# graphdeco-inria/nerfshop

Hardware: AMD Instinct MI355X
Metric: render_msamples_per_s_1080p (higher is better)
Workload: dtype f16 storage / f32 accumulate (MFMA), f32 marching+compositing; 1 GPU; lego-like snapshot 1920x1080, one cage edit (BASELINE configs[2]/[4]); samples_per_frame=25213758, frames_in_flight=1, cell_records=levels 0..11, 9.2 GB (nrs_model_set_cell_cache default)

## Files before the change

nerfshop_amd/csrc/nrs_api_edit.cpp:

```cpp
#include "nrs_host.h"

#include <cmath>
#include <cstdio>
#include <cstring>
#include <limits>
#include <memory>
#include <new>

using namespace nrs;

static void box_of(const float* v, uint32_t n, Box3& b) {
	const float inf = std::numeric_limits<float>::infinity();
	for (int k = 0; k < 3; ++k) { b.mn[k] = inf; b.mx[k] = -inf; }
	for (uint32_t i = 0; i < n; ++i)
		for (int k = 0; k < 3; ++k) {
			b.mn[k] = std::fmin(b.mn[k], v[3 * i + k]);
			b.mx[k] = std::fmax(b.mx[k], v[3 * i + k]);
		}
}
static void warp_box(const Box3& b, const Box3& aabb, Box3& out) {
	for (int k = 0; k < 3; ++k) {
		const float diag = aabb.mx[k] - aabb.mn[k];
		out.mn[k] = (b.mn[k] - aabb.mn[k]) / diag;
		out.mx[k] = (b.mx[k] - aabb.mn[k]) / diag;
// ... 78 lines not shown
			for (int a = 0; a < 3; ++a) { f[a] = w[a] << shift; f[4 + a] = (w[3 + a] - w[a] + 1) << shift; }
			f[7] = shift;
			budget -= cells;
			base += (uint32_t)cells;
			any = true;
			break;
		}
	}
	if (!any) { memset(de.fine_win, 0, sizeof(de.fine_win)); return NRS_OK; }
	const uint32_t n_cells = base, n_padded = (n_cells + 4095u) / 4096u * 4096u;
	if (n_padded > e->fine_cells_cap || (want_head && !e->d_fine_head.get())) {
		e->d_fine_off.reset(); e->d_fine_counts.reset(); e->d_fine_head.reset();
		e->fine_cells_cap = 0;
		const size_t cap = std::min<size_t>(kFineMaxCells, (size_t)n_padded + n_padded / 4 + 4095) / 4096 * 4096;
		HIP_TRY(e->d_fine_off.alloc(cap + 1));
		HIP_TRY(e->d_fine_counts.alloc(cap));
		if (want_head) HIP_TRY(e->d_fine_head.alloc(cap));
		e->fine_cells_cap = cap;
	}
	NRS_LAUNCH(launch_fine_count_scan(de, n_cells, e->d_fine_counts.get(), e->d_fine_tiles.get(), e->d_fine_off.get(), (uint32_t*)e->d_fine_win.get() + kCascades * 8, s));
	uint32_t n_idx = 0;
	HIP_TRY(hipMemcpyAsync(&n_idx, e->d_fine_win.get() + kCascades * 8, 4, hipMemcpyDeviceToHost, s));
	HIP_TRY(hipStreamSynchronize(s));
	if ((size_t)n_idx > e->fine_idx_cap || !e->d_fine_idx.get()) {
		e->d_fine_idx.reset();
		e->fine_idx_cap = 0;
		const size_t cap = std::max<size_t>((size_t)n_idx + n_idx / 2, 1024);
		HIP_TRY(e->d_fine_idx.alloc(cap));
		e->fine_idx_cap = cap;
	}
	NRS_LAUNCH(launch_fine_fill(de, n_cells, e->d_fine_off.get(), e->d_fine_idx.get(), want_head ? e->d_fine_head.get() : nullptr, s));
	e->fine_n_idx = n_idx;
	de.fine_off = e->d_fine_off.get();
	de.fine_idx = e->d_fine_idx.get();
	de.fine_head = want_head ? e->d_fine_head.get() : nullptr;
	static const bool log_fine = dev_knob("NRS_FINE_LOG") != nullptr;
	if (log_fine) fprintf(stderr, "[nrs fine lut] %u fine cells, %u entries (the LUT holds %u), subdivision per cascade %d %d %d %d %d, head words %s\n", n_cells, n_idx, e->lut_n_idx, de.fine_win[0][7],
	                      de.fine_win[1][7], de.fine_win[2][7], de.fine_win[3][7], de.fine_win[4][7], de.fine_head ? "yes" : "no");
	return NRS_OK;
}
static int rebuild_after_vertices(nrs_edit* e, hipStream_t s, bool build_fine_now = false) {
	NRS_TRY(ensure_build_scratch(e));
	NRS_LAUNCH(launch_bbox(e->n_vertices, e->d_verts.get(), (float*)e->d_scratch.get(), s));
	NRS_TRY(build_lut_on_device(e, e->d_verts.get(), nullptr, s));
	if (e->d_rot.get()) NRS_LAUNCH(launch_local_rotations(e->n_tets, e->d_verts.get(), e->de.orig, e->de.tets, e->d_rot.get(), e->d_mapback.get(), s));
	NRS_LAUNCH(launch_tet_planes(e->n_tets, e->d_verts.get(), e->de.tets, e->d_planes.get(), s));
	if (build_fine_now) NRS_TRY(build_fine_lut(e, s));
	else {
		e->de.fine_off = nullptr;
		e->de.fine_idx = nullptr;
		e->de.fine_head = nullptr;
		memset(e->de.fine_win, 0, sizeof(e->de.fine_win));
		e->fine_stale = true;
		e->renders_since_move = 0;
	}
	uint32_t host[8];
	HIP_TRY(hipMemcpyAsync(host, e->d_scratch.get(), sizeof(host), hipMemcpyDeviceToHost, s));
	HIP_TRY(hipStreamSynchronize(s));
	memcpy(e->de.bbox.mn, host, 12);
	memcpy(e->de.bbox.mx, host + 3, 12);
	warp_box(e->de.bbox, e->de.aabb, e->de.warped_bbox);
// ... 283 lines not shown
```

nerfshop_amd/csrc/nrs_api_render.cpp:

```cpp
#include "nrs_host.h"

#include <array>
#include <cmath>
#include <cstdio>
#include <cstdlib>
#include <cstring>

using namespace nrs;

extern "C" {

static int tile_geometry(const nrs_render_params& p, uint32_t team, uint32_t& tiles_x, uint32_t& owned, uint32_t& n_packets, uint32_t& ppt_x) {
	const uint32_t W = (uint32_t)p.resolution[0], H = (uint32_t)p.resolution[1];
	const uint32_t pw = team >= 16 ? 2u : (team >= 4 ? 4u : 8u), ph = 64u / team / pw;
	if (p.tile_size == 0) {
		tiles_x = (W + pw - 1) / pw;
		owned = 1;
		ppt_x = 0;
		n_packets = tiles_x * ((H + ph - 1) / ph);
		return NRS_OK;
	}
	if (p.tile_size % 8) return fail(NRS_ERR_INVALID_ARG, "tile_size must be a multiple of 8");
	tiles_x = tile_pitch(W, p.tile_size);
	const uint32_t tiles_y = (H + p.tile_size - 1) / p.tile_size, total = tiles_x * tiles_y;
// ... 173 lines not shown
		}
		ctx->counters_clean[slot] = true;
	}
	HIP_TRY(hipEventRecord(ctx->slot_done[slot], s));
	ctx->slot_stream[slot] = s;
	ctx->slot_used[slot] = true;
	return NRS_OK;
}

static int report_wave_log(nrs_ctx* ctx, const RenderCounters& c) {
	static const char* names[8] = {"fill", "refill", "setup+warp", "gather", "sh+mlp", "composite+march+shade", "-", "exit"};
	unsigned long long tot = 0;
	for (int i = 0; i < 8; ++i) if (i != 6) tot += c.phase_cycles[i];
	fprintf(stderr, "[nrs phases] samples=%llu", (unsigned long long)c.n_samples);
	for (int i = 0; i < 8; ++i)
		if (c.phase_cycles[i] && i != 6) fprintf(stderr, " %s=%.1f%%", names[i], 100.0 * (double)c.phase_cycles[i] / (double)tot);
	fprintf(stderr, " | mean wave lifetime = %.1f%% of the longest (%.2f Mcycles)", 100.0 * ((double)tot / 4096.0) / (double)c.phase_cycles[6], (double)c.phase_cycles[6] / 1e6);
	fprintf(stderr, "\n");
	fprintf(stderr, "[nrs walk] fill: %llu lane iterations in %llu wave trips (%.1f lanes busy per trip); march: %llu lane iterations in %llu wave trips "
	        "(%.1f lanes/trip), %llu of %llu rounds needed > 1 trip; live lanes per round %.1f\n",
	        c.walk[0], c.walk[1], c.walk[1] ? (double)c.walk[0] / (double)c.walk[1] : 0.0, c.walk[2], c.walk[3],
	        c.walk[3] ? (double)c.walk[2] / (double)c.walk[3] : 0.0, c.walk[6], c.walk[4], c.walk[4] ? (double)c.walk[5] / (double)c.walk[4] : 0.0);
	if (c.walk[8])
		fprintf(stderr, "[nrs cage scan] %llu samples inside a deformed box (%.1f %% of the samples), %llu of them found a tet; rounds with such a sample: %llu of %llu (%.1f %%); "
		        "candidates tested %llu (%.2f per sample in the box), scan wave trips %llu (%.2f per round that scans)\n",
		        c.walk[8], 100.0 * (double)c.walk[8] / (double)std::max<unsigned long long>(c.n_samples, 1), c.walk[12], c.walk[9], c.walk[4], 100.0 * (double)c.walk[9] / (double)std::max<unsigned long long>(c.walk[4], 1),
		        c.walk[10], (double)c.walk[10] / (double)c.walk[8], c.walk[11], (double)c.walk[11] / (double)std::max<unsigned long long>(c.walk[9], 1));
	std::vector<unsigned long long> wl(8192 * 4);
	HIP_TRY(hipMemcpy(wl.data(), ctx->d_wave_log.get(), wl.size() * 8, hipMemcpyDeviceToHost));
	if (const char* dump = dev_knob("NRS_WAVE_LOG_FILE")) {
		if (FILE* f = fopen(dump, "wb")) { fwrite(wl.data(), 8, wl.size(), f); fclose(f); }
	}
	std::vector<std::array<unsigned long long, 4>> rec;
	unsigned long long t0min = ~0ull;
	for (size_t i = 0; i < 8192; ++i) if (wl[4 * i]) t0min = std::min(t0min, wl[4 * i + 3] >> 32);
	for (size_t i = 0; i < 8192; ++i)
		if (wl[4 * i]) {
			const unsigned long long wall = wl[4 * i + 3] & 0xffffffffull, start = (wl[4 * i + 3] >> 32) - t0min;
			const unsigned long long rq = (wl[4 * i + 1] >> 16) & 0xffff, tq = (wl[4 * i + 1] >> 32) + start;
			rec.push_back({wall + start, (wl[4 * i + 1] & 0xffffull) | (rq << 16) | (tq << 32), wl[4 * i + 2] & 0xffffull, wl[4 * i + 2] >> 56});
		}
	std::sort(rec.begin(), rec.end());
	if (!rec.empty()) {
		auto pr = [&](const char* tag, size_t i) {
			fprintf(stderr, "   %s: end=%.1f us, queue found empty at %.1f us, rounds=%llu (%llu after that), packets=%llu, xcc=%llu\n", tag, rec[i][0] / 100.0,
			        (rec[i][1] >> 32) / 100.0, rec[i][1] & 0xffff, (rec[i][1] & 0xffff) - ((rec[i][1] >> 16) & 0xffff), rec[i][2], rec[i][3]);
		};
		double mean = 0;
		for (auto& r : rec) mean += (double)r[0];
// ... 154 lines not shown
```

nerfshop_amd/csrc/nrs_cage.hip:

```cpp
#include <hip/hip_runtime.h>
#include "nrs_internal.h"
#include "nrs_launch.h"
#include "nrs_device.cuh"
#include "nrs_scan.cuh"
#include "nrs_svd3.h"

namespace nrs {


constexpr uint32_t kCells = kGridVol * kCascades;
constexpr uint32_t kScanTile = 4096;
static_assert(kCells % kScanTile == 0, "scan tiles must cover the cell array exactly");
constexpr uint32_t kScanTiles = kCells / kScanTile;
static_assert(kFineMaxCells % kScanTile == 0 && kFineScanTiles == kFineMaxCells / kScanTile, "fine look-up table: scan tiles");

__global__ void mvc_apply_kernel(uint32_t n_points, uint32_t n_cv, const float* __restrict__ weights, const float* __restrict__ cage,
                                 float* __restrict__ points) {
	const uint32_t i = blockIdx.x * blockDim.x + threadIdx.x;
	if (i >= n_points) return;
	f3 p = mk3(0.f, 0.f, 0.f);
	const float* w = weights + (size_t)i * n_cv;
	for (uint32_t v = 0; v < n_cv; ++v) {
		const float wv = w[v];
		p = p + mk3(wv * cage[3 * v], wv * cage[3 * v + 1], wv * cage[3 * v + 2]);
	}
	points[3 * i] = p.x; points[3 * i + 1] = p.y; points[3 * i + 2] = p.z;
}

// ... 393 lines not shown
	float R[9];
	svd3::tet_rotation(o, d, R);
	for (int k = 0; k < 9; ++k) out[9 * (size_t)i + k] = R[k];
	if (mapback)
		for (int k = 0; k < 9; ++k) mapback[24 * (size_t)i + 12 + k] = R[k];
}
__global__ void tet_mapback_kernel(uint32_t n_tets, const float* __restrict__ org, const uint32_t* __restrict__ tets, const float* __restrict__ rot, float* __restrict__ mapback) {
	const uint32_t i = blockIdx.x * blockDim.x + threadIdx.x;
	if (i >= n_tets) return;
	const uint4 tv = reinterpret_cast<const uint4*>(tets)[i];
	const f3 v[4] = {ld3(org, tv.x), ld3(org, tv.y), ld3(org, tv.z), ld3(org, tv.w)};
	float out[24];
	for (int f = 0; f < 4; ++f) { out[3 * f] = v[f].x; out[3 * f + 1] = v[f].y; out[3 * f + 2] = v[f].z; }
	for (int k = 0; k < 9; ++k) out[12 + k] = rot ? rot[9 * (size_t)i + k] : 0.f;
	for (int k = 21; k < 24; ++k) out[k] = 0.f;
	float4* dst = reinterpret_cast<float4*>(mapback) + 6 * (size_t)i;
	for (int q = 0; q < 6; ++q) dst[q] = make_float4(out[4 * q], out[4 * q + 1], out[4 * q + 2], out[4 * q + 3]);
}

__global__ void tet_planes_kernel(uint32_t n_tets, const float* __restrict__ verts, const uint32_t* __restrict__ tets, float* __restrict__ planes) {
	const uint32_t i = blockIdx.x * blockDim.x + threadIdx.x;
	if (i >= n_tets) return;
	const uint4 tv = reinterpret_cast<const uint4*>(tets)[i];
	const f3 v[4] = {ld3(verts, tv.x), ld3(verts, tv.y), ld3(verts, tv.z), ld3(verts, tv.w)};
	float out[32];
	uint32_t signs = 0;
	for (int f = 0; f < 4; ++f) {
		const f3 v1 = v[f], v2 = v[(f + 1) & 3], v3 = v[(f + 2) & 3], v4 = v[(f + 3) & 3];
		const f3 normal = cross3(v2 - v1, v3 - v1);
		const float dotV4 = dot3(normal, v4 - v1);
		out[3 * f] = v1.x; out[3 * f + 1] = v1.y; out[3 * f + 2] = v1.z;
		out[12 + 3 * f] = normal.x; out[12 + 3 * f + 1] = normal.y; out[12 + 3 * f + 2] = normal.z;
		signs |= (__float_as_uint(dotV4) >> 31) << f;
	}
	out[24] = __uint_as_float(signs);
	for (int k = 25; k < 32; ++k) out[k] = 0.f;
	float4* dst = reinterpret_cast<float4*>(planes) + 8 * (size_t)i;
	for (int q = 0; q < 8; ++q) dst[q] = make_float4(out[4 * q], out[4 * q + 1], out[4 * q + 2], out[4 * q + 3]);
}

__global__ __launch_bounds__(256) void fine_window_kernel(const uint32_t* __restrict__ offsets, int32_t* __restrict__ win) {
	__shared__ int32_t red[8];
	if (threadIdx.x < 8) red[threadIdx.x] = threadIdx.x < 3 ? 0x7fffffff : (threadIdx.x < 6 ? -1 : 0);
	__syncthreads();
	const uint32_t first = (blockIdx.x * blockDim.x + threadIdx.x) * 16u;
	uint32_t o[17];
	#pragma unroll
	for (int q = 0; q < 4; ++q) { const uint4 v = reinterpret_cast<const uint4*>(offsets + first)[q]; o[4 * q] = v.x; o[4 * q + 1] = v.y; o[4 * q + 2] = v.z; o[4 * q + 3] = v.w; }
	o[16] = offsets[first + 16];
	if (o[0] != o[16]) {
		int32_t lo[3] = {0x7fffffff, 0x7fffffff, 0x7fffffff}, hi[3] = {-1, -1, -1}, cells = 0, longest = 0;
		#pragma unroll
		for (uint32_t k = 0; k < 16; ++k) {
			if (o[k + 1] != o[k]) {
				const uint32_t m = (first + k) % kGridVol;
				const int32_t c[3] = {(int32_t)morton3D_invert(m), (int32_t)morton3D_invert(m >> 1), (int32_t)morton3D_invert(m >> 2)};
				for (int a = 0; a < 3; ++a) { lo[a] = min(lo[a], c[a]); hi[a] = max(hi[a], c[a]); }
				++cells;
				longest = max(longest, (int32_t)(o[k + 1] - o[k]));
			}
		}
		for (int a = 0; a < 3; ++a) { atomicMin(&red[a], lo[a]); atomicMax(&red[3 + a], hi[a]); }
		atomicAdd(&red[6], cells);
		atomicMax(&red[7], longest);
	}
	__syncthreads();
	if (threadIdx.x < 8 && red[6] != 0) {
		int32_t* dst = win + (blockIdx.x * blockDim.x * 16u / kGridVol) * 8 + threadIdx.x;
		if (threadIdx.x < 3) atomicMin(dst, red[threadIdx.x]);
		else if (threadIdx.x < 6 || threadIdx.x == 7) atomicMax(dst, red[threadIdx.x]);
		else atomicAdd(dst, red[6]);
	}
}
__device__ __forceinline__ bool tet_may_contain_box(const float* __restrict__ r, const float c[3], const float h[3]) {
	const uint32_t signs = __float_as_uint(r[24]);
	bool may = true;
	#pragma unroll
	for (int f = 0; f < 4; ++f) {
		float dc = 0.f, rad = 0.f, err = 0.f;
		#pragma unroll
		for (int i = 0; i < 3; ++i) {
			const float n = r[12 + 3 * f + i], d = c[i] - r[3 * f + i];
			dc = fmaf(n, d, dc);
			rad = fmaf(fabsf(n), h[i], rad);
			err = fmaf(fabsf(n), fabsf(d) + h[i], err);
		}
		const float slack = fmaf(err, 20.0f / 16777216.0f, 1e-30f);
		may = may && (((signs >> f) & 1u) ? !(dc - rad > slack) : !(dc + rad < -slack));
	}
	return may;
}
template <bool FILL>
__global__ __launch_bounds__(256) void fine_lists_kernel(const DeviceEdit e, uint32_t* __restrict__ counts, const uint32_t* __restrict__ fine_off,
                                                         uint32_t* __restrict__ fine_idx, uint2* __restrict__ fine_head) {
	uint32_t w = blockIdx.x * (blockDim.x >> 6) + (threadIdx.x >> 6);
	const uint32_t lane = threadIdx.x & 63u;
	uint32_t level = kCascades;
	#pragma unroll
	for (uint32_t c = 0; c < kCascades; ++c) {
		const int32_t* f = e.fine_win[c];
		const uint32_t n_par = (f[4] == 0 || (uint32_t)f[7] > 2u) ? 0u : ((uint32_t)f[4] >> f[7]) * ((uint32_t)f[5] >> f[7]) * ((uint32_t)f[6] >> f[7]);
		if (level == kCascades) { if (w < n_par) level = c; else w -= n_par; }
	}
	if (level == kCascades) return;
	const uint32_t S = (uint32_t)e.fine_win[level][7], sub = 1u << S;
	const uint32_t ex = (uint32_t)e.fine_win[level][4], ey = (uint32_t)e.fine_win[level][5];
	const uint32_t px = ex >> S, py = ey >> S;
	const uint32_t cx = w % px, cy = (w / px) % py, cz = w / (px * py);
	const uint32_t lx = ((uint32_t)e.fine_win[level][0] >> S) + cx, ly = ((uint32_t)e.fine_win[level][1] >> S) + cy, lz = ((uint32_t)e.fine_win[level][2] >> S) + cz;
	const uint32_t parent = level * kGridVol + morton3D(lx, ly, lz);
	const uint32_t j0 = e.lut_off[parent], j1 = e.lut_off[parent + 1];
	const bool owner = lane < sub * sub * sub;
	const uint32_t sx = lane & (sub - 1u), sy = (lane >> S) & (sub - 1u), sz = lane >> (2u * S);
	const uint32_t rx = (cx << S) + sx, ry = (cy << S) + sy, rz = (cz << S) + sz;
	const uint32_t cell = (uint32_t)e.fine_win[level][3] + (rz * ey + ry) * ex + rx;
	if (j0 == j1) {
		if (!FILL && owner) counts[cell] = 0u;
		if (FILL && owner && fine_head) fine_head[cell] = make_uint2(0u, 0u);
		return;
	}
	const uint32_t res = kGrid << S;
	const double scale = (double)(1u << level), margin = 2e-6 * scale;
	const uint32_t f[3] = {(uint32_t)e.fine_win[level][0] + rx, (uint32_t)e.fine_win[level][1] + ry, (uint32_t)e.fine_win[level][2] + rz};
	float c[3], h[3];
	bool border = false;
	#pragma unroll
	for (int i = 0; i < 3; ++i) {
		const double lo = 0.5 + ((double)f[i] / (double)res - 0.5) * scale - margin, hi = 0.5 + ((double)(f[i] + 1) / (double)res - 0.5) * scale + margin;
		c[i] = (float)(0.5 * (lo + hi));
		h[i] = (float)(0.5 * (hi - lo));
		border = border || f[i] == 0 || f[i] >= res - 1;
	}
	uint32_t n = 0, wpos = (FILL && owner) ? fine_off[cell] : 0u;
	const uint32_t wpos0 = wpos;
	uint32_t first = 0u;
	for (uint32_t b = j0; b < j1; b += 64u) {
		const uint32_t mine = b + lane < j1 ? e.lut_idx[b + lane] : 0u;
		const uint32_t nb = min(64u, j1 - b);
		float4 cur[7], nxt[7];
		{
			const float4* q = reinterpret_cast<const float4*>(e.planes) + 8 * (size_t)(uint32_t)__builtin_amdgcn_readlane((int)mine, 0);
			#pragma unroll
			for (int i = 0; i < 7; ++i) cur[i] = q[i];
		}
		for (uint32_t k = 0; k < nb; ++k) {
			const uint32_t t = (uint32_t)__builtin_amdgcn_readlane((int)mine, (int)k);
			const uint32_t t_next = (uint32_t)__builtin_amdgcn_readlane((int)mine, (int)min(k + 1u, nb - 1u));
			{
				const float4* q = reinterpret_cast<const float4*>(e.planes) + 8 * (size_t)t_next;
				#pragma unroll
				for (int i = 0; i < 7; ++i) nxt[i] = q[i];
			}
			const float* r = reinterpret_cast<const float*>(cur);
			if ((border || tet_may_contain_box(r, c, h)) && owner) {
				if (FILL) { fine_idx[wpos++] = t; if (n == 0) first = t; }
				++n;
			}
			#pragma unroll
			for (int i = 0; i < 7; ++i) cur[i] = nxt[i];
		}
	}
	if (!FILL && owner) counts[cell] = n;
	if (FILL && owner && fine_head) fine_head[cell] = make_uint2(wpos0, first | (n << kFineHeadTetBits));
}

int launch_mvc_apply(uint32_t n_points, uint32_t n_cv, const float* d_weights, const float* d_cage, float* d_points, void* stream) {
	hipLaunchKernelGGL(mvc_apply_kernel, dim3((n_points + 127) / 128), dim3(128), 0, (hipStream_t)stream, n_points, n_cv, d_weights, d_cage, d_points);
	NRS_LAUNCH_CHECK("mvc_apply_kernel launch");
	return NRS_OK;
}
int launch_poisson_interpolate(uint32_t n_points, uint32_t n_cv, const float* d_gamma, const float* d_per_cage, float* d_shs, float* d_out_density, float* d_res_density, void* stream) {
	hipLaunchKernelGGL(poisson_interpolate_kernel, dim3((n_points + 63) / 64), dim3(64), 0, (hipStream_t)stream, n_points, n_cv, d_gamma, d_per_cage, d_shs, d_out_density, d_res_density);
	NRS_LAUNCH_CHECK("poisson_interpolate_kernel launch");
	return NRS_OK;
}
int launch_bbox(uint32_t n, const float* d_verts, float* d_out6, void* stream) {
	hipLaunchKernelGGL(bbox_kernel, dim3(1), dim3(256), 0, (hipStream_t)stream, n, d_verts, d_out6);
	NRS_LAUNCH_CHECK("bbox_kernel launch");
	return NRS_OK;
}
int launch_lut_count_scan(uint32_t n_tets, const float* d_verts, const uint32_t* d_tets, uint32_t* d_counts, uint32_t* d_tile_sums,
                          uint32_t* d_offsets, uint32_t* d_total, unsigned long long* d_hit_masks, float cells0, void* stream) {
	hipStream_t s = (hipStream_t)stream;
	launch_tet_mark<false>(n_tets, cells0, d_verts, d_tets, d_counts, nullptr, nullptr, d_hit_masks, s);
	const int status = launch_cell_scan(kScanTiles, d_counts, d_tile_sums, d_offsets, d_total, s);
	if (status != NRS_OK) return status;
// ... 71 lines not shown
```

nerfshop_amd/csrc/nrs_device.cuh:

```cuda
#pragma once
#include <hip/hip_runtime.h>
#include "nrs_internal.h"

namespace nrs {

struct f3 { float x, y, z; };
__device__ __forceinline__ f3 mk3(float x, float y, float z) { return f3{x, y, z}; }
__device__ __forceinline__ f3 operator+(f3 a, f3 b) { return {a.x + b.x, a.y + b.y, a.z + b.z}; }
__device__ __forceinline__ f3 operator-(f3 a, f3 b) { return {a.x - b.x, a.y - b.y, a.z - b.z}; }
__device__ __forceinline__ f3 operator*(f3 a, float s) { return {a.x * s, a.y * s, a.z * s}; }
__device__ __forceinline__ f3 operator*(float s, f3 a) { return {s * a.x, s * a.y, s * a.z}; }
__device__ __forceinline__ float sum3(float a, float b, float c) { return a + (b + c); }
__device__ __forceinline__ float dot3(f3 a, f3 b) { return sum3(a.x * b.x, a.y * b.y, a.z * b.z); }
__device__ __forceinline__ f3 mat3_mul(const float* M, f3 v) {
	return {sum3(M[0] * v.x, M[3] * v.y, M[6] * v.z), sum3(M[1] * v.x, M[4] * v.y, M[7] * v.z), sum3(M[2] * v.x, M[5] * v.y, M[8] * v.z)};
}
__device__ __forceinline__ f3 cross3(f3 a, f3 b) { return {a.y * b.z - a.z * b.y, a.z * b.x - a.x * b.z, a.x * b.y - a.y * b.x}; }

__device__ __forceinline__ bool box_contains(const Box3& b, f3 p) {
	return p.x >= b.mn[0] && p.x <= b.mx[0] && p.y >= b.mn[1] && p.y <= b.mx[1] && p.z >= b.mn[2] && p.z <= b.mx[2];
}

#define NRS_SQRT3 1.73205080757f
#define NRS_MIN_STEP (NRS_SQRT3 / 1024)
#define NRS_MAX_STEP (NRS_MIN_STEP * (1 << (kCascades - 1)) * 1024 / kGrid)
// ... 574 lines not shown
	       same_side_tet(v4, v1, v2, v3, p);
}
__device__ __forceinline__ void bary_tet(f3 a, f3 b, f3 c, f3 d, f3 p, float out[4]) {
	f3 vap = p - a, vbp = p - b, vab = b - a, vac = c - a, vad = d - a, vbc = c - b, vbd = d - b;
	float va6 = scalar_tp(vbp, vbd, vbc);
	float vb6 = scalar_tp(vap, vac, vad);
	float vc6 = scalar_tp(vap, vad, vab);
	float vd6 = scalar_tp(vap, vab, vac);
	float v6 = (float)(1. / (double)scalar_tp(vab, vac, vad));
	out[0] = va6 * v6; out[1] = vb6 * v6; out[2] = vc6 * v6; out[3] = vd6 * v6;
}
template <typename T>
__device__ __forceinline__ const NRS_GLOBAL T* gp(const T* p) { return (const NRS_GLOBAL T*)p; }
__device__ __forceinline__ f3 ld3(const float* __restrict__ a, uint32_t i) {
	typedef float f3a __attribute__((ext_vector_type(3), aligned(4)));
	const f3a v = *(const NRS_GLOBAL f3a*)(gp(a) + 3 * (size_t)i);
	return {v.x, v.y, v.z};
}

__device__ __forceinline__ bool point_in_tet_rec(const float* __restrict__ recs, uint32_t t, f3 p) {
	typedef float f4n __attribute__((ext_vector_type(4)));
	const NRS_GLOBAL f4n* q = gp(reinterpret_cast<const f4n*>(recs)) + 8 * (size_t)t;
	const f4n v0 = q[0], v1 = q[1], v2 = q[2], n0 = q[3], n1 = q[4], n2 = q[5], sg = q[6];
	const float d0 = dot3(mk3(n0.x, n0.y, n0.z), p - mk3(v0.x, v0.y, v0.z));
	const float d1 = dot3(mk3(n0.w, n1.x, n1.y), p - mk3(v0.w, v1.x, v1.y));
	const float d2 = dot3(mk3(n1.z, n1.w, n2.x), p - mk3(v1.z, v1.w, v2.x));
	const float d3 = dot3(mk3(n2.y, n2.z, n2.w), p - mk3(v2.y, v2.z, v2.w));
	const uint32_t got = (__float_as_uint(d0) >> 31) | ((__float_as_uint(d1) >> 31) << 1) | ((__float_as_uint(d2) >> 31) << 2) | ((__float_as_uint(d3) >> 31) << 3);
	return got == __float_as_uint(sg.x);
}
__device__ __forceinline__ uint32_t scan_entries_for_tet(const DeviceEdit& e, const NRS_GLOBAL uint32_t* lut_idx, uint32_t j0, uint32_t j1, uint32_t t, f3 p, uint32_t* n_tested) {
	uint32_t found = 0xffffffffu;
	#pragma unroll 1
	for (uint32_t j = j0; j < j1; ++j) {
		const uint32_t t_next = lut_idx[min(j + 1, j1 - 1)];
		if (n_tested) ++*n_tested;
		if (point_in_tet_rec(e.planes, t, p)) { found = t; break; }
		t = t_next;
	}
	return found;
}
__device__ __forceinline__ uint32_t scan_list_for_tet(const DeviceEdit& e, const uint32_t* __restrict__ off, const uint32_t* __restrict__ idx, uint32_t cell, f3 p, uint32_t* n_tested = nullptr) {
	const NRS_GLOBAL uint32_t* lut_off = gp(off);
	const NRS_GLOBAL uint32_t* lut_idx = gp(idx);
	const uint32_t j0 = lut_off[cell], j1 = lut_off[cell + 1];
	if (j0 >= j1) return 0xffffffffu;
	return scan_entries_for_tet(e, lut_idx, j0, j1, lut_idx[j0], p, n_tested);
}
__device__ __forceinline__ uint32_t scan_cell_for_tet(const DeviceEdit& e, uint32_t cell, f3 p, uint32_t* n_tested = nullptr) { return scan_list_for_tet(e, e.lut_off, e.lut_idx, cell, p, n_tested); }
__device__ __forceinline__ uint32_t scan_fine_cell_for_tet(const DeviceEdit& e, uint32_t cell, f3 p, uint32_t* n_tested = nullptr) {
	typedef uint32_t u2n __attribute__((ext_vector_type(2)));
	const u2n head = *reinterpret_cast<const NRS_GLOBAL u2n*>(gp(e.fine_head) + cell);
	const uint32_t n = head.y >> kFineHeadTetBits;
	return scan_entries_for_tet(e, gp(e.fine_idx), head.x, head.x + n, head.y & ((1u << kFineHeadTetBits) - 1u), p, n_tested);
}
template <bool SHORT = true>
__device__ __forceinline__ uint32_t find_tet(const DeviceEdit& e, f3 u, const uint32_t* __restrict__ march_lds, uint32_t* n_tested = nullptr) {
	const int level = mip_from_pos(u);
	if (e.fine_off) {
		typedef int32_t i4n __attribute__((ext_vector_type(4)));
		i4n lo, ext;
		const int level_u = __builtin_amdgcn_readfirstlane(level);
		if (SHORT && __all(level == level_u)) {
			const NRS_CONSTANT i4n* win = (const NRS_CONSTANT i4n*)reinterpret_cast<const i4n*>(&e.fine_win[0][0]) + 2 * level_u;
			lo = win[0]; ext = win[1];
		} else {
			const NRS_GLOBAL i4n* win = gp(reinterpret_cast<const i4n*>(&e.fine_win[0][0])) + 2 * level;
			lo = win[0]; ext = win[1];
		}
		const float mip_scale = ldexpf(1.0f, -level);
		f3 q = u - mk3(0.5f, 0.5f, 0.5f);
		q = q * mip_scale;
		q = q + mk3(0.5f, 0.5f, 0.5f);
		if (ext.w != kFinePlain) {
			const int fres_i = (int)(kGrid << ext.w);
			const float fres = (float)fres_i;
			const int hi = fres_i - 1;
// ... 57 lines not shown
				f4n r0 = {0.f, 0.f, 0.f, 0.f}, r1 = {0.f, 0.f, 0.f, 0.f};
				float r2 = 0.f;
				if (rotate) { r0 = mq[3]; r1 = mq[4]; r2 = reinterpret_cast<const NRS_GLOBAL float*>(mq)[20]; }
				f3 canon = bc[0] * mk3(o0.x, o0.y, o0.z) + bc[1] * mk3(o0.w, o1.x, o1.y);
				canon = canon + bc[2] * mk3(o1.z, o1.w, o2.x);
				canon = canon + bc[3] * mk3(o2.y, o2.z, o2.w);
				wpos = e.diag_pow2 ? mk3((canon.x - e.aabb.mn[0]) * e.inv_diag[0], (canon.y - e.aabb.mn[1]) * e.inv_diag[1], (canon.z - e.aabb.mn[2]) * e.inv_diag[2])
				                   : warp_position(canon, e.aabb);
				if (rotate) {
					const f3 ud = unwarp_direction(wdir);
					const float R[9] = {r0.x, r0.y, r0.z, r0.w, r1.x, r1.y, r1.z, r1.w, r2};
					const f3 rd = mat3_mul(R, ud);
					wdir = warp_direction(rd);
				}
			}
			in_deformed = true;
		}
	}
	bool empty = false;
	if (!(with_dir && e.copy)) {
		if (!in_deformed && box_contains(e.orig_warped_bbox, wpos)) {
			const f3 u = unwarp_position(wpos, e.aabb);
			const int level = mip_from_pos(u);
			const uint32_t pos_idx = cascaded_grid_idx_at(u, (uint32_t)level);
			empty = gp(e.orig_bitfield)[pos_idx / 8 + (kGridVol * (uint32_t)level) / 8] & (1 << (pos_idx % 8));
		}
	}
	return empty;
}

__device__ __forceinline__ bool affine_contains(const AffineBox& b, f3 p) {
	const f3 q = p - mk3(b.mn[0], b.mn[1], b.mn[2]);
	const float du = dot3(mk3(b.u[0], b.u[1], b.u[2]), q), dv = dot3(mk3(b.v[0], b.v[1], b.v[2]), q), dw = dot3(mk3(b.w[0], b.w[1], b.w[2]), q);
	return du >= 0.f && du < b.uu && dv >= 0.f && dv < b.vv && dw >= 0.f && dw < b.ww;
}
__device__ __forceinline__ f3 mul_rt(const float* R, f3 q) {
	return {sum3(R[0] * q.x, R[1] * q.y, R[2] * q.z), sum3(R[3] * q.x, R[4] * q.y, R[5] * q.z), sum3(R[6] * q.x, R[7] * q.y, R[8] * q.z)};
}
__device__ __forceinline__ bool affine_warp(const DeviceEdit& e, bool with_dir, f3& wpos, f3& wdir) {
	if (affine_contains(e.a_dst, wpos)) {
		const f3 c = mk3(e.a_dst.center[0], e.a_dst.center[1], e.a_dst.center[2]);
		const f3 d = wpos - c;
		const f3 q = {d.x / e.a_scale[0], d.y / e.a_scale[1], d.z / e.a_scale[2]};
		f3 p = mul_rt(e.a_rot, q) + c;
		wpos = p - mk3(e.a_translation[0], e.a_translation[1], e.a_translation[2]);
		if (with_dir && e.a_correct_dir) wdir = warp_direction(mul_rt(e.a_rot, unwarp_direction(wdir)));
		return false;
	}
// ... 243 lines not shown
```

nerfshop_amd/csrc/nrs_internal.h:

```cpp
#pragma once
#include <stdint.h>
#include <stddef.h>
#include "../../include/nrs.h"
#include "nrs_route.h"

#include <stdlib.h>
#include <hip/hip_vector_types.h>

namespace nrs {

inline const char* dev_knob(const char* name) {
	static const bool on = []() { const char* e = getenv("NRS_DEV_KNOBS"); return e && e[0] && e[0] != '0'; }();
	return on ? getenv(name) : nullptr;
}

constexpr uint32_t kGrid = 128;
constexpr uint32_t kCascades = 5;
constexpr uint32_t kGridVol = kGrid * kGrid * kGrid;
constexpr uint32_t kLevels = 16;
constexpr uint32_t kCoarse = 32;
constexpr uint32_t kCoarseWords = kCoarse * kCoarse * kCoarse / 32;
static_assert((kCoarse & (kCoarse - 1)) == 0, "the block walk's bounds test (cx | cy | cz) needs a power of two");
constexpr uint32_t kDensityW = 64 * 32 + 16 * 64;
constexpr uint32_t kRgbW = 64 * 32 + 64 * 64 + 16 * 64;
// ... 181 lines not shown
int launch_map_rays(const DeviceEdit& e, uint32_t n, float* d_coords, uint32_t ld, int with_dir, uint8_t* d_empty, void* stream);
int launch_grid_to_bitfield(const float* d_grid, uint8_t* d_bitfield, float* d_scratch_mean, void* stream);
int launch_occ_accel(const uint8_t* d_bitfield, uint32_t* d_masks, float* d_out, uint32_t* d_keys, void* stream);
int launch_grid_update(const DeviceModel& m, const DeviceEdit* d_edits, int n_edits, const nrs_grid_update& u, uint64_t rng_state_nonuniform,
                       float* d_grid, uint32_t* d_grid_tmp, int n_cus, void* stream);
int launch_accumulate(uint32_t n_pixels, const float* d_frame, float* d_accum, uint32_t sample_count, int color_space, void* stream);
int launch_accumulate_spp(uint32_t n_pixels, const float* d_frames, size_t slab_stride_pixels, uint32_t spp_count, float* d_accum, uint32_t sample_count, int color_space, void* stream);
int launch_tonemap(uint32_t n_pixels, const float* d_accum, const nrs_tonemap_params& p, void* d_out, void* stream);
int launch_accumulate_spp_tonemap(uint32_t n_pixels, const float* d_frames, size_t slab_stride_pixels, uint32_t spp_count, float* d_accum, uint32_t sample_count,
                                  const nrs_tonemap_params& p, void* d_out, void* stream);
int launch_detile(const nrs_render_params& p, uint32_t n_ranks, size_t rank_stride_floats, const float* d_tiles, uint32_t channels,
                  float* d_image, void* stream);
const char* launch_last_error();

int launch_tile_scan(uint32_t n_tiles, uint32_t n_values, uint32_t* d_sums, uint32_t* d_totals, uint32_t* d_total_copy, void* stream);

constexpr uint32_t kLutScanTiles = kGridVol * kCascades / 4096;
constexpr uint32_t kFineMaxCells = 16u << 20;
constexpr uint32_t kFineScanTiles = kFineMaxCells / 4096;
constexpr int32_t kFinePlain = 0xff;
constexpr int32_t kFineMaxList = 96;
constexpr uint32_t kFineHeadTetBits = 25;
static_assert(kFineMaxList < (1 << (32 - kFineHeadTetBits)), "a fine list (a filtered LUT list of at most kFineMaxList tets) must fit the head word's length field");
int launch_mvc_apply(uint32_t n_points, uint32_t n_cv, const float* d_weights, const float* d_cage, float* d_points, void* stream);
int launch_bbox(uint32_t n, const float* d_verts, float* d_out6, void* stream);
int launch_poisson_interpolate(uint32_t n_points, uint32_t n_cv, const float* d_gamma, const float* d_per_cage, float* d_shs, float* d_out_density, float* d_res_density, void* stream);
int launch_lut_count_scan(uint32_t n_tets, const float* d_verts, const uint32_t* d_tets, uint32_t* d_counts, uint32_t* d_tile_sums,
                          uint32_t* d_offsets, uint32_t* d_total, unsigned long long* d_hit_masks ,
                          float cells0 , void* stream);
int launch_lut_fill(uint32_t n_tets, const float* d_verts, const uint32_t* d_tets, uint32_t* d_counts, const uint32_t* d_offsets, uint32_t* d_idx,
                    uint8_t* d_bitfield, uint32_t* d_scratch_u32 , uint32_t* d_big_cells, uint32_t n_work , unsigned long long* d_hit_masks , float cells0, void* stream);
uint32_t lut_big_list_capacity(size_t idx_capacity);
int launch_tet_planes(uint32_t n_tets, const float* d_verts, const uint32_t* d_tets, float* d_planes, void* stream);
int launch_fine_window(const uint32_t* d_lut_off, int32_t* d_window_out, void* stream);
int launch_fine_count_scan(const DeviceEdit& de, uint32_t n_fine_cells, uint32_t* d_counts, uint32_t* d_tile_sums, uint32_t* d_fine_off, uint32_t* d_total, void* stream);
int launch_fine_fill(const DeviceEdit& de, uint32_t n_fine_cells, const uint32_t* d_fine_off, uint32_t* d_fine_idx, uint2* d_fine_head , void* stream);
int launch_local_rotations(uint32_t n_tets, const float* d_verts, const float* d_orig, const uint32_t* d_tets, float* d_out, float* d_mapback, void* stream);
int launch_tet_mapback(uint32_t n_tets, const float* d_orig, const uint32_t* d_tets, const float* d_rot, float* d_mapback, void* stream);

constexpr uint32_t kMcBlock = 256;
constexpr uint32_t kMcRowCap = 32;
struct McGrid {
	uint32_t res[3];
	uint32_t n;
	float scale[3], offset[3];
	float thresh;
// ... 37 lines not shown
```

nerfshop_amd/csrc/nrs_render.cuh:

```cuda
#pragma once
#include <hip/hip_runtime.h>
#include "nrs_internal.h"
#include "nrs_device.cuh"
#include "nrs_mlp.cuh"

namespace nrs {

__device__ __forceinline__ uint32_t lds_peek(const uint32_t* p) { return __atomic_load_n(p, __ATOMIC_RELAXED); }
__device__ __forceinline__ void lds_poke(uint32_t* p, uint32_t v) { __atomic_store_n(p, v, __ATOMIC_RELAXED); }
constexpr int kRing = 128;
constexpr int kTeamMax = 4;
#ifndef NRS_MEASURE
#define NRS_MEASURE 0
#endif
constexpr uint32_t kRefillWhenIdle = 64;

template <int WAVES>
struct RenderSmem {
	ModelLds ml;
	FeatLds fl[WAVES];
	uint2 ring[WAVES][kRing];
	uint32_t coarse[kMarchLdsWords];
	unsigned long long queue;
	unsigned long long sum_samples;
// ... 460 lines not shown
		if (ops && act) {
#if NRS_MEASURE == 2
			{ f3 wp2 = wpos, wd2 = wdir; asm volatile("" : "+v"(wp2.x), "+v"(wp2.y), "+v"(wp2.z)); bool e2 = false;
			  for (int ei = a2.n_edits - 1; ei >= 0; --ei) e2 |= AFFINE ? edit_warp<!POISSON>(a2.edits[ei], true, wp2, wd2) : tet_warp<!POISSON && GATE == 0, GATE == 0>(a2.edits[ei], true, wp2, wd2);
			  asm volatile("" :: "v"(wp2.x), "v"(wp2.y), "v"(wp2.z), "v"(wd2.x), "v"(wd2.y), "v"(wd2.z), "s"((int)__ballot(e2))); }
#endif
			for (int ei = a2.n_edits - 1; ei >= 0; --ei) {
				if (AFFINE) {
					empty |= edit_warp<!POISSON>(a2.edits[ei], true, wpos, wdir);
				} else if (POISSON) {
					uint32_t scan;
					empty |= tet_warp<false>(a2.edits[ei], true, wpos, wdir, sm.coarse, &scan);
					if (ei == a2.n_edits - 1) warp_scan = scan;
				} else {
					empty |= tet_warp<GATE == 0, GATE == 0>(a2.edits[ei], true, wpos, wdir, sm.coarse, nullptr, PROF ? &pf_scan : nullptr);
				}
			}
		}
		if (PROF && !POISSON && !AFFINE) {
			uint32_t mx = pf_scan & 0xffffu;
			for (int sh = 32; sh > 0; sh >>= 1) mx = max(mx, (uint32_t)__shfl_xor((int)mx, sh, 64));
			pf_walk[8] += (pf_scan >> 16) & 1u; pf_walk[9] += (lane == 0 && __any((pf_scan >> 16) & 1u)) ? 1u : 0u;
			pf_walk[10] += pf_scan & 0xffffu; pf_walk[11] += (lane == 0) ? mx : 0u; pf_walk[12] += (pf_scan >> 17) & 1u;
		}
		if (POISSON && !AFFINE) poisson_stash[wave * 64 + lane] = warp_scan;
		NRS_PHASE(3);
#if NRS_MEASURE == 3
		{ f3 wp2 = wpos; asm volatile("" : "+v"(wp2.x), "+v"(wp2.y), "+v"(wp2.z));
		  encode_num<NUM, kQuads>(nm, gv, m2.levels, sm.ml, fl, lane, g, wp2, act); }
#endif
		encode_num<NUM, kQuads, false, GATE>(nm, gv, m2.levels, sm.ml, fl, lane, g, wpos, act);
		NRS_PHASE(4);
		const f3 pdir = mk3(xchg32(wdir.x), xchg32(wdir.y), xchg32(wdir.z));
		half8 sh_own, sh_par;
		encode_sh4_2(g, wdir, pdir, sh_own, sh_par);

#if NRS_MEASURE == 4
		{ uint32_t sink = 0;
		  #pragma unroll 1
		  for (int b = 0; b < 2; ++b) {
			const int sel = (b != g) ? 1 : 0;
			half8 x0 = load_features(fl, lane, sel, 0), x1 = load_features(fl, lane, sel, 1);
			asm volatile("" : "+v"(x0), "+v"(x1));
			const half8 dout = density_mlp_num<NUM>(nm, sm.ml.w, lane, x0, x1);
			const half8 rout = rgb_mlp_num<NUM>(nm, sm.ml.w, lane, dout, sel ? sh_par : sh_own);
			sink ^= __builtin_bit_cast(u32x4, dout)[0] ^ __builtin_bit_cast(u32x4, rout)[1];
// ... 377 lines not shown
```

Baseline: 13290 Msamples/s.

## Mark fine cells fully inside one tet as proven and skip the per-sample tet scan

While building the fine LUT, each tet is classified against the cell box as cannot/may/must-contain. When the first listed tet provably contains the whole cell, the head word stores a sentinel, and the render-time lookup returns that tet without testing any candidates. This removes the point-in-tet scans for samples in such cells, at the cost of a slightly more expensive build pass and a conservative floating-point slack argument. The change also routes the original-bitfield occupancy lookup through the LDS march table when one is available, and adds logging counters.

```diff
diff --git a/nerfshop_amd/csrc/nrs_api_edit.cpp b/nerfshop_amd/csrc/nrs_api_edit.cpp
--- a/nerfshop_amd/csrc/nrs_api_edit.cpp
+++ b/nerfshop_amd/csrc/nrs_api_edit.cpp
@@ -124,6 +124,7 @@
 	uint32_t n_idx = 0;
 	HIP_TRY(hipMemcpyAsync(&n_idx, e->d_fine_win.get() + kCascades * 8, 4, hipMemcpyDeviceToHost, s));
 	HIP_TRY(hipStreamSynchronize(s));
+	if (n_idx >= kFineHeadProven) return fail(NRS_ERR_INVALID_ARG, "fine look-up table: more entries than a head word can address");
 	if ((size_t)n_idx > e->fine_idx_cap || !e->d_fine_idx.get()) {
 		e->d_fine_idx.reset();
 		e->fine_idx_cap = 0;
@@ -137,8 +138,17 @@
 	de.fine_idx = e->d_fine_idx.get();
 	de.fine_head = want_head ? e->d_fine_head.get() : nullptr;
 	static const bool log_fine = dev_knob("NRS_FINE_LOG") != nullptr;
-	if (log_fine) fprintf(stderr, "[nrs fine lut] %u fine cells, %u entries (the LUT holds %u), subdivision per cascade %d %d %d %d %d, head words %s\n", n_cells, n_idx, e->lut_n_idx, de.fine_win[0][7],
-	                      de.fine_win[1][7], de.fine_win[2][7], de.fine_win[3][7], de.fine_win[4][7], de.fine_head ? "yes" : "no");
+	if (log_fine) {
+		uint32_t listed = 0, proven = 0;
+		if (de.fine_head) {
+			std::vector<uint2> heads(n_cells);
+			HIP_TRY(hipMemcpyAsync(heads.data(), de.fine_head, (size_t)n_cells * sizeof(uint2), hipMemcpyDeviceToHost, s));
+			HIP_TRY(hipStreamSynchronize(s));
+			for (const uint2& h : heads) { listed += (h.y >> kFineHeadTetBits) != 0u; proven += h.x == kFineHeadProven; }
+		}
+		fprintf(stderr, "[nrs fine lut] %u fine cells, %u entries (the LUT holds %u), subdivision per cascade %d %d %d %d %d, proven cells %u of %u with a list, head words %s\n", n_cells, n_idx,
+		        e->lut_n_idx, de.fine_win[0][7], de.fine_win[1][7], de.fine_win[2][7], de.fine_win[3][7], de.fine_win[4][7], proven, listed, de.fine_head ? "yes" : "no");
+	}
 	return NRS_OK;
 }
 static int rebuild_after_vertices(nrs_edit* e, hipStream_t s, bool build_fine_now = false) {
diff --git a/nerfshop_amd/csrc/nrs_api_render.cpp b/nerfshop_amd/csrc/nrs_api_render.cpp
--- a/nerfshop_amd/csrc/nrs_api_render.cpp
+++ b/nerfshop_amd/csrc/nrs_api_render.cpp
@@ -219,9 +219,10 @@
 	        c.walk[0], c.walk[1], c.walk[1] ? (double)c.walk[0] / (double)c.walk[1] : 0.0, c.walk[2], c.walk[3],
 	        c.walk[3] ? (double)c.walk[2] / (double)c.walk[3] : 0.0, c.walk[6], c.walk[4], c.walk[4] ? (double)c.walk[5] / (double)c.walk[4] : 0.0);
 	if (c.walk[8])
-		fprintf(stderr, "[nrs cage scan] %llu samples inside a deformed box (%.1f %% of the samples), %llu of them found a tet; rounds with such a sample: %llu of %llu (%.1f %%); "
-		        "candidates tested %llu (%.2f per sample in the box), scan wave trips %llu (%.2f per round that scans)\n",
-		        c.walk[8], 100.0 * (double)c.walk[8] / (double)std::max<unsigned long long>(c.n_samples, 1), c.walk[12], c.walk[9], c.walk[4], 100.0 * (double)c.walk[9] / (double)std::max<unsigned long long>(c.walk[4], 1),
+		fprintf(stderr, "[nrs cage scan] %llu samples inside a deformed box (%.1f %% of the samples), %llu of them found a tet, %llu (%.1f %%) with no candidate tested; "
+		        "rounds with such a sample: %llu of %llu (%.1f %%); candidates tested %llu (%.2f per sample in the box), scan wave trips %llu (%.2f per round that scans)\n",
+		        c.walk[8], 100.0 * (double)c.walk[8] / (double)std::max<unsigned long long>(c.n_samples, 1), c.walk[12] & 0xffffffffull, c.walk[12] >> 32,
+		        100.0 * (double)(c.walk[12] >> 32) / (double)c.walk[8], c.walk[9], c.walk[4], 100.0 * (double)c.walk[9] / (double)std::max<unsigned long long>(c.walk[4], 1),
 		        c.walk[10], (double)c.walk[10] / (double)c.walk[8], c.walk[11], (double)c.walk[11] / (double)std::max<unsigned long long>(c.walk[9], 1));
 	std::vector<unsigned long long> wl(8192 * 4);
 	HIP_TRY(hipMemcpy(wl.data(), ctx->d_wave_log.get(), wl.size() * 8, hipMemcpyDeviceToHost));
diff --git a/nerfshop_amd/csrc/nrs_cage.hip b/nerfshop_amd/csrc/nrs_cage.hip
--- a/nerfshop_amd/csrc/nrs_cage.hip
+++ b/nerfshop_amd/csrc/nrs_cage.hip
@@ -4,6 +4,7 @@
 #include "nrs_device.cuh"
 #include "nrs_scan.cuh"
 #include "nrs_svd3.h"
+#include "nrs_tet_box.h"
 
 namespace nrs {
 
@@ -443,19 +444,10 @@
 	const uint32_t i = blockIdx.x * blockDim.x + threadIdx.x;
 	if (i >= n_tets) return;
 	const uint4 tv = reinterpret_cast<const uint4*>(tets)[i];
-	const f3 v[4] = {ld3(verts, tv.x), ld3(verts, tv.y), ld3(verts, tv.z), ld3(verts, tv.w)};
+	const f3 p[4] = {ld3(verts, tv.x), ld3(verts, tv.y), ld3(verts, tv.z), ld3(verts, tv.w)};
+	const float v[4][3] = {{p[0].x, p[0].y, p[0].z}, {p[1].x, p[1].y, p[1].z}, {p[2].x, p[2].y, p[2].z}, {p[3].x, p[3].y, p[3].z}};
 	float out[32];
-	uint32_t signs = 0;
-	for (int f = 0; f < 4; ++f) {
-		const f3 v1 = v[f], v2 = v[(f + 1) & 3], v3 = v[(f + 2) & 3], v4 = v[(f + 3) & 3];
-		const f3 normal = cross3(v2 - v1, v3 - v1);
-		const float dotV4 = dot3(normal, v4 - v1);
-		out[3 * f] = v1.x; out[3 * f + 1] = v1.y; out[3 * f + 2] = v1.z;
-		out[12 + 3 * f] = normal.x; out[12 + 3 * f + 1] = normal.y; out[12 + 3 * f + 2] = normal.z;
-		signs |= (__float_as_uint(dotV4) >> 31) << f;
-	}
-	out[24] = __uint_as_float(signs);
-	for (int k = 25; k < 32; ++k) out[k] = 0.f;
+	tet_plane_record(v, out);
 	float4* dst = reinterpret_cast<float4*>(planes) + 8 * (size_t)i;
 	for (int q = 0; q < 8; ++q) dst[q] = make_float4(out[4 * q], out[4 * q + 1], out[4 * q + 2], out[4 * q + 3]);
 }
@@ -492,24 +484,6 @@
 		else if (threadIdx.x < 6 || threadIdx.x == 7) atomicMax(dst, red[threadIdx.x]);
 		else atomicAdd(dst, red[6]);
 	}
-}
-__device__ __forceinline__ bool tet_may_contain_box(const float* __restrict__ r, const float c[3], const float h[3]) {
-	const uint32_t signs = __float_as_uint(r[24]);
-	bool may = true;
-	#pragma unroll
-	for (int f = 0; f < 4; ++f) {
-		float dc = 0.f, rad = 0.f, err = 0.f;
-		#pragma unroll
-		for (int i = 0; i < 3; ++i) {
-			const float n = r[12 + 3 * f + i], d = c[i] - r[3 * f + i];
-			dc = fmaf(n, d, dc);
-			rad = fmaf(fabsf(n), h[i], rad);
-			err = fmaf(fabsf(n), fabsf(d) + h[i], err);
-		}
-		const float slack = fmaf(err, 20.0f / 16777216.0f, 1e-30f);
-		may = may && (((signs >> f) & 1u) ? !(dc - rad > slack) : !(dc + rad < -slack));
-	}
-	return may;
 }
 template <bool FILL>
 __global__ __launch_bounds__(256) void fine_lists_kernel(const DeviceEdit e, uint32_t* __restrict__ counts, const uint32_t* __restrict__ fine_off,
@@ -555,6 +529,7 @@
 	uint32_t n = 0, wpos = (FILL && owner) ? fine_off[cell] : 0u;
 	const uint32_t wpos0 = wpos;
 	uint32_t first = 0u;
+	bool proven = false;
 	for (uint32_t b = j0; b < j1; b += 64u) {
 		const uint32_t mine = b + lane < j1 ? e.lut_idx[b + lane] : 0u;
 		const uint32_t nb = min(64u, j1 - b);
@@ -573,8 +548,9 @@
 				for (int i = 0; i < 7; ++i) nxt[i] = q[i];
 			}
 			const float* r = reinterpret_cast<const float*>(cur);
-			if ((border || tet_may_contain_box(r, c, h)) && owner) {
-				if (FILL) { fine_idx[wpos++] = t; if (n == 0) first = t; }
+			const uint32_t cls = border ? kTetBoxMay : tet_box_classify(r, c, h);
+			if (cls != kTetBoxCannot && owner) {
+				if (FILL) { fine_idx[wpos++] = t; if (n == 0) { first = t; proven = cls == kTetBoxMust; } }
 				++n;
 			}
 			#pragma unroll
@@ -582,7 +558,7 @@
 		}
 	}
 	if (!FILL && owner) counts[cell] = n;
-	if (FILL && owner && fine_head) fine_head[cell] = make_uint2(wpos0, first | (n << kFineHeadTetBits));
+	if (FILL && owner && fine_head) fine_head[cell] = make_uint2(proven ? kFineHeadProven : wpos0, first | (n << kFineHeadTetBits));
 }
 
 int launch_mvc_apply(uint32_t n_points, uint32_t n_cv, const float* d_weights, const float* d_cage, float* d_points, void* stream) {
diff --git a/nerfshop_amd/csrc/nrs_device.cuh b/nerfshop_amd/csrc/nrs_device.cuh
--- a/nerfshop_amd/csrc/nrs_device.cuh
+++ b/nerfshop_amd/csrc/nrs_device.cuh
@@ -1,6 +1,7 @@
 #pragma once
 #include <hip/hip_runtime.h>
 #include "nrs_internal.h"
+#include "nrs_tet_box.h"
 
 namespace nrs {
 
@@ -621,12 +622,8 @@
 	typedef float f4n __attribute__((ext_vector_type(4)));
 	const NRS_GLOBAL f4n* q = gp(reinterpret_cast<const f4n*>(recs)) + 8 * (size_t)t;
 	const f4n v0 = q[0], v1 = q[1], v2 = q[2], n0 = q[3], n1 = q[4], n2 = q[5], sg = q[6];
-	const float d0 = dot3(mk3(n0.x, n0.y, n0.z), p - mk3(v0.x, v0.y, v0.z));
-	const float d1 = dot3(mk3(n0.w, n1.x, n1.y), p - mk3(v0.w, v1.x, v1.y));
-	const float d2 = dot3(mk3(n1.z, n1.w, n2.x), p - mk3(v1.z, v1.w, v2.x));
-	const float d3 = dot3(mk3(n2.y, n2.z, n2.w), p - mk3(v2.y, v2.z, v2.w));
-	const uint32_t got = (__float_as_uint(d0) >> 31) | ((__float_as_uint(d1) >> 31) << 1) | ((__float_as_uint(d2) >> 31) << 2) | ((__float_as_uint(d3) >> 31) << 3);
-	return got == __float_as_uint(sg.x);
+	const float r[25] = {v0.x, v0.y, v0.z, v0.w, v1.x, v1.y, v1.z, v1.w, v2.x, v2.y, v2.z, v2.w, n0.x, n0.y, n0.z, n0.w, n1.x, n1.y, n1.z, n1.w, n2.x, n2.y, n2.z, n2.w, sg.x};
+	return tet_rec_contains(r, p.x, p.y, p.z);
 }
 __device__ __forceinline__ uint32_t scan_entries_for_tet(const DeviceEdit& e, const NRS_GLOBAL uint32_t* lut_idx, uint32_t j0, uint32_t j1, uint32_t t, f3 p, uint32_t* n_tested) {
 	uint32_t found = 0xffffffffu;
@@ -650,8 +647,9 @@
 __device__ __forceinline__ uint32_t scan_fine_cell_for_tet(const DeviceEdit& e, uint32_t cell, f3 p, uint32_t* n_tested = nullptr) {
 	typedef uint32_t u2n __attribute__((ext_vector_type(2)));
 	const u2n head = *reinterpret_cast<const NRS_GLOBAL u2n*>(gp(e.fine_head) + cell);
-	const uint32_t n = head.y >> kFineHeadTetBits;
-	return scan_entries_for_tet(e, gp(e.fine_idx), head.x, head.x + n, head.y & ((1u << kFineHeadTetBits) - 1u), p, n_tested);
+	const uint32_t n = head.y >> kFineHeadTetBits, first = head.y & ((1u << kFineHeadTetBits) - 1u);
+	if (head.x == kFineHeadProven) return first;
+	return scan_entries_for_tet(e, gp(e.fine_idx), head.x, head.x + n, first, p, n_tested);
 }
 template <bool SHORT = true>
 __device__ __forceinline__ uint32_t find_tet(const DeviceEdit& e, f3 u, const uint32_t* __restrict__ march_lds, uint32_t* n_tested = nullptr) {
@@ -755,8 +753,8 @@
 		if (!in_deformed && box_contains(e.orig_warped_bbox, wpos)) {
 			const f3 u = unwarp_position(wpos, e.aabb);
 			const int level = mip_from_pos(u);
-			const uint32_t pos_idx = cascaded_grid_idx_at(u, (uint32_t)level);
-			empty = gp(e.orig_bitfield)[pos_idx / 8 + (kGridVol * (uint32_t)level) / 8] & (1 << (pos_idx % 8));
+			const uint32_t bit_idx = march_lds ? occupancy_bit_index(u, (uint32_t)level, march_lds) : (uint32_t)level * kGridVol + cascaded_grid_idx_at(u, (uint32_t)level);
+			empty = gp(e.orig_bitfield)[bit_idx / 8] & (1 << (bit_idx % 8));
 		}
 	}
 	return empty;
diff --git a/nerfshop_amd/csrc/nrs_internal.h b/nerfshop_amd/csrc/nrs_internal.h
--- a/nerfshop_amd/csrc/nrs_internal.h
+++ b/nerfshop_amd/csrc/nrs_internal.h
@@ -227,6 +227,8 @@
 constexpr int32_t kFineMaxList = 96;
 constexpr uint32_t kFineHeadTetBits = 25;
 static_assert(kFineMaxList < (1 << (32 - kFineHeadTetBits)), "a fine list (a filtered LUT list of at most kFineMaxList tets) must fit the head word's length field");
+constexpr uint32_t kFineHeadProven = 0xffffffffu;
+static_assert((uint64_t)kFineMaxCells * (uint64_t)kFineMaxList < (uint64_t)kFineHeadProven, "no fine list may start at kFineHeadProven: fine_idx holds at most kFineMaxCells lists of at most kFineMaxList tets");
 int launch_mvc_apply(uint32_t n_points, uint32_t n_cv, const float* d_weights, const float* d_cage, float* d_points, void* stream);
 int launch_bbox(uint32_t n, const float* d_verts, float* d_out6, void* stream);
 int launch_poisson_interpolate(uint32_t n_points, uint32_t n_cv, const float* d_gamma, const float* d_per_cage, float* d_shs, float* d_out_density, float* d_res_density, void* stream);
diff --git a/nerfshop_amd/csrc/nrs_render.cuh b/nerfshop_amd/csrc/nrs_render.cuh
--- a/nerfshop_amd/csrc/nrs_render.cuh
+++ b/nerfshop_amd/csrc/nrs_render.cuh
@@ -506,6 +506,7 @@
 			for (int sh = 32; sh > 0; sh >>= 1) mx = max(mx, (uint32_t)__shfl_xor((int)mx, sh, 64));
 			pf_walk[8] += (pf_scan >> 16) & 1u; pf_walk[9] += (lane == 0 && __any((pf_scan >> 16) & 1u)) ? 1u : 0u;
 			pf_walk[10] += pf_scan & 0xffffu; pf_walk[11] += (lane == 0) ? mx : 0u; pf_walk[12] += (pf_scan >> 17) & 1u;
+			if ((pf_scan & 0x2ffffu) == 0x20000u) pf_walk[12] += 1ull << 32;
 		}
 		if (POISSON && !AFFINE) poisson_stash[wave * 64 + lane] = warp_scan;
 		NRS_PHASE(3);
diff --git a/nerfshop_amd/csrc/nrs_tet_box.h b/nerfshop_amd/csrc/nrs_tet_box.h
--- /dev/null
+++ b/nerfshop_amd/csrc/nrs_tet_box.h
@@ -0,0 +1,74 @@
+#pragma once
+#include <math.h>
+#include <stdint.h>
+#include <string.h>
+
+#if defined(__HIPCC__)
+#define NRS_TET_BOX_FN __host__ __device__ __forceinline__
+#else
+#define NRS_TET_BOX_FN inline
+#endif
+
+namespace nrs {
+
+NRS_TET_BOX_FN uint32_t tet_box_float_bits(float v) {
+	uint32_t u;
+	memcpy(&u, &v, 4);
+	return u;
+}
+NRS_TET_BOX_FN void tet_plane_record(const float v[4][3], float out[32]) {
+	uint32_t signs = 0;
+	for (int f = 0; f < 4; ++f) {
+		const float* v1 = v[f];
+		const float* v2 = v[(f + 1) & 3];
+		const float* v3 = v[(f + 2) & 3];
+		const float* v4 = v[(f + 3) & 3];
+		const float a[3] = {v2[0] - v1[0], v2[1] - v1[1], v2[2] - v1[2]}, b[3] = {v3[0] - v1[0], v3[1] - v1[1], v3[2] - v1[2]}, d[3] = {v4[0] - v1[0], v4[1] - v1[1], v4[2] - v1[2]};
+		const float n[3] = {a[1] * b[2] - a[2] * b[1], a[2] * b[0] - a[0] * b[2], a[0] * b[1] - a[1] * b[0]};
+		const float dot_v4 = n[0] * d[0] + (n[1] * d[1] + n[2] * d[2]);
+		for (int i = 0; i < 3; ++i) { out[3 * f + i] = v1[i]; out[12 + 3 * f + i] = n[i]; }
+		signs |= (tet_box_float_bits(dot_v4) >> 31) << f;
+	}
+	memcpy(&out[24], &signs, 4);
+	for (int k = 25; k < 32; ++k) out[k] = 0.f;
+}
+NRS_TET_BOX_FN float tet_face_dot(const float* r, int f, float px, float py, float pz) {
+	const float dx = px - r[3 * f], dy = py - r[3 * f + 1], dz = pz - r[3 * f + 2];
+	return r[12 + 3 * f] * dx + (r[12 + 3 * f + 1] * dy + r[12 + 3 * f + 2] * dz);
+}
+NRS_TET_BOX_FN bool tet_rec_contains(const float* r, float px, float py, float pz) {
+	const uint32_t got = (tet_box_float_bits(tet_face_dot(r, 0, px, py, pz)) >> 31) | ((tet_box_float_bits(tet_face_dot(r, 1, px, py, pz)) >> 31) << 1) |
+	                     ((tet_box_float_bits(tet_face_dot(r, 2, px, py, pz)) >> 31) << 2) | ((tet_box_float_bits(tet_face_dot(r, 3, px, py, pz)) >> 31) << 3);
+	return got == tet_box_float_bits(r[24]);
+}
+
+enum : uint32_t { kTetBoxCannot = 0u, kTetBoxMay = 1u, kTetBoxMust = 3u };
+NRS_TET_BOX_FN uint32_t tet_box_classify(const float* r, const float c[3], const float h[3]) {
+	const uint32_t signs = tet_box_float_bits(r[24]);
+	bool may = true, must = true;
+#if defined(__HIPCC__)
+	#pragma unroll
+#endif
+	for (int f = 0; f < 4; ++f) {
+		float dc = 0.f, rad = 0.f, err = 0.f;
+#if defined(__HIPCC__)
+		#pragma unroll
+#endif
+		for (int i = 0; i < 3; ++i) {
+			const float n = r[12 + 3 * f + i], d = c[i] - r[3 * f + i];
+			dc = fmaf(n, d, dc);
+			rad = fmaf(fabsf(n), h[i], rad);
+			err = fmaf(fabsf(n), fabsf(d) + h[i], err);
+		}
+		const float slack = fmaf(err, 20.0f / 16777216.0f, 1e-30f);
+		const bool all_positive = dc - rad > slack, all_negative = dc + rad < -slack;
+		const bool want_negative = ((signs >> f) & 1u) != 0u;
+		may = may && !(want_negative ? all_positive : all_negative);
+		must = must && (want_negative ? all_negative : all_positive);
+	}
+	return may ? (must ? kTetBoxMust : kTetBoxMay) : kTetBoxCannot;
+}
+NRS_TET_BOX_FN bool tet_may_contain_box(const float* r, const float c[3], const float h[3]) { return tet_box_classify(r, c, h) != kTetBoxCannot; }
+NRS_TET_BOX_FN bool tet_must_contain_box(const float* r, const float c[3], const float h[3]) { return tet_box_classify(r, c, h) == kTetBoxMust; }
+
+}
```

Result: no change. 13270 Msamples/s (-0.2%).
